# bergmanlab/TELR

Measured on AMD Instinct MI355X. Metric: gbp_aligned_per_s, higher is better.
Workload: dtype int16

## Files before the change

telr_amd/_lib.py:

```python
import ctypes as C
import os
from ._abi import IdxOpt, MapOpt, Aln, Counters, N_STAGES

os.environ.setdefault("GPU_MAX_HW_QUEUES", "2")
_HERE = os.path.dirname(os.path.abspath(__file__))
SO_PATH = os.environ.get("TELR_LIB") or os.path.join(_HERE, "libtelrhip.so")

EXPORTS = [
    "telr_init", "telr_destroy", "telr_strerror", "telr_last_error", "telr_device_name", "telr_preset",
    "telr_seqset_create", "telr_seqset_subset", "telr_seqset_subset_rc", "telr_seqset_free", "telr_seqset_bases", "telr_seqset_count",
    "telr_index_build", "telr_index_free", "telr_index_stats", "telr_map",
    "telr_result_from_arrays", "telr_result_count", "telr_result_alns", "telr_result_cigar_count", "telr_result_cigars", "telr_result_wait", "telr_result_free",
    "telr_init_background", "telr_release_scratch", "telr_device_mem", "telr_write_paf", "telr_write_sam", "telr_write_bam", "telr_write_bam_dev", "telr_bam_prepare", "telr_bam_release_wait", "telr_bam_discard", "telr_write_bam_slice", "telr_bam_segment_info", "telr_bam_segment_entries", "telr_bam_segment_write", "telr_bam_segment_free", "telr_bai_write", "telr_result_from_device_cigars", "telr_seqset_packed", "telr_seqset_from_packed", "telr_consensus_build", "telr_poa_build", "telr_consensus_count", "telr_consensus_seq", "telr_consensus_off", "telr_consensus_len", "telr_consensus_free", "telr_fasta_load", "telr_fasta_count", "telr_fasta_bases", "telr_fasta_extent", "telr_fasta_seq", "telr_fasta_off", "telr_fasta_len", "telr_fasta_names", "telr_fasta_free", "telr_depth_medians", "telr_window_reads", "telr_stage_ms", "telr_stage_name", "telr_last_counters", "telr_last_dp_classes",
]

_lib = None


class TelrError(RuntimeError):
    def __init__(self, msg, code=None):
        RuntimeError.__init__(self, msg)
        self.code = code


# ... 57 lines not shown
        getattr(L, fn).restype = vp; getattr(L, fn).argtypes = [vp]
    L.telr_consensus_free.restype = None; L.telr_consensus_free.argtypes = [vp]
    L.telr_bam_prepare.restype = C.c_int; L.telr_bam_prepare.argtypes = [vp, cp, i64]
    L.telr_bam_release_wait.restype = C.c_int; L.telr_bam_release_wait.argtypes = []
    L.telr_bam_discard.restype = C.c_int; L.telr_bam_discard.argtypes = [vp]
    L.telr_write_bam_slice.restype = C.c_int; L.telr_write_bam_slice.argtypes = [vp, vp, vp, vp, vp, vp, i32, cp, cp, cp, cp, vp, i32, i32, C.POINTER(vp)]
    L.telr_bam_segment_info.restype = C.c_int; L.telr_bam_segment_info.argtypes = [vp, vp]
    L.telr_bam_segment_entries.restype = C.c_int; L.telr_bam_segment_entries.argtypes = [vp, i64, vp, vp, vp, vp, vp]
    L.telr_bam_segment_write.restype = C.c_int; L.telr_bam_segment_write.argtypes = [vp, vp, cp, i64, i32]
    L.telr_bam_segment_free.restype = None; L.telr_bam_segment_free.argtypes = [vp]
    L.telr_bai_write.restype = C.c_int; L.telr_bai_write.argtypes = [cp, i64, vp, vp, vp, vp, C.c_uint64, i64, i32, vp]
    L.telr_result_from_device_cigars.restype = C.c_int; L.telr_result_from_device_cigars.argtypes = [vp, vp, i64, vp, i64, C.POINTER(vp)]
    L.telr_debug_bam_twin.restype = C.c_int; L.telr_debug_bam_twin.argtypes = []
    L.telr_debug_result_twin.restype = i64; L.telr_debug_result_twin.argtypes = [vp, vp, i64]
    L.telr_debug_bam_sink_ms.restype = C.c_int; L.telr_debug_bam_sink_ms.argtypes = [vp]
    L.telr_debug_bam_ms.restype = C.c_int; L.telr_debug_bam_ms.argtypes = [vp]
    L.telr_debug_huff.restype = C.c_int; L.telr_debug_huff.argtypes = [vp, i32, i32, vp]
    L.telr_debug_check_records.restype = C.c_int; L.telr_debug_check_records.argtypes = [vp, i64, vp, i64, vp, i32, vp, i32, C.POINTER(i64)]
    L.telr_debug_deflate_host.restype = C.c_int; L.telr_debug_deflate_host.argtypes = [vp, i32, vp, i32, vp]
    L.telr_stage_ms.restype = C.c_int; L.telr_stage_ms.argtypes = [vp, vp]
    L.telr_stage_name.restype = cp; L.telr_stage_name.argtypes = [C.c_int]
    L.telr_last_counters.restype = C.c_int; L.telr_last_counters.argtypes = [vp, C.POINTER(Counters)]
    L.telr_last_dp_classes.restype = C.c_int; L.telr_last_dp_classes.argtypes = [vp, vp]
    L.telr_debug_n_anchor.restype = i64; L.telr_debug_n_anchor.argtypes = [vp]
    L.telr_debug_dp_retries.restype = i64; L.telr_debug_dp_retries.argtypes = [vp]
    L.telr_debug_pk_launches.restype = i64; L.telr_debug_pk_launches.argtypes = [vp]
    L.telr_debug_fetch.restype = C.c_int; L.telr_debug_fetch.argtypes = [vp, cp, vp, i64]
    L.telr_debug_n_chain.restype = i64; L.telr_debug_n_chain.argtypes = [vp]
    L.telr_debug_chains.restype = vp; L.telr_debug_chains.argtypes = [vp]
    L.telr_debug_index.restype = C.c_int; L.telr_debug_index.argtypes = [vp, vp, vp, vp, vp]
    L.telr_debug_pack.restype = C.c_int; L.telr_debug_pack.argtypes = [cp, i32, C.c_int, vp, vp]
    L.telr_debug_mid_occ.restype = i32; L.telr_debug_mid_occ.argtypes = [vp, C.POINTER(MapOpt)]
    L.telr_debug_dp_limits.restype = C.c_int; L.telr_debug_dp_limits.argtypes = [C.POINTER(MapOpt), vp]
    L.telr_debug_dp.restype = C.c_int; L.telr_debug_dp.argtypes = [vp, vp, vp, C.POINTER(MapOpt), vp, i32, vp, vp, vp, i64]
    L.telr_debug_chain.restype = C.c_int; L.telr_debug_chain.argtypes = [vp, i32, vp, vp, C.POINTER(MapOpt), vp, vp]
    _lib = L
    return L
```

telr_amd/csrc/kernels.hip.h:

```cpp
#pragma once
#include <hip/hip_runtime.h>
#include <stdint.h>

#define TELR_NEG      (-(1 << 28))
#define TELR_TPAD     16384
#define SK_TILE       1024
#define SK_THREADS    256
#define DP_DMAX       4096

struct ChainOpt {
    int32_t max_gap, bw, min_cnt, min_chain_score, chain_gap_q8, chain_skip_q8;
    int32_t dense_n, dense_span, mw_n;
};
struct DpOpt {
    int32_t a, b, q, e, q2, e2, sc_ambi, zdrop;
    int32_t cx_scale, cx_open, cx_emax, cx_emin, cx_dec, cx_flat;
};
__host__ __device__ __forceinline__ int d_cx_ext(const DpOpt &o, int len) { int v = o.cx_emax - o.cx_dec * len; return v > o.cx_emin ? v : o.cx_emin; }
__host__ __device__ __forceinline__ int d_cx_cost(const DpOpt &o, int L)
{
    int t = o.cx_open;
    for (int i = 0; i < L && i < o.cx_flat; ++i) t += d_cx_ext(o, i);
    if (L > o.cx_flat) t += (L - o.cx_flat) * o.cx_emin;
    return t;
// ... 2014 lines not shown
        if (D <= 128) return 6;
        if (D <= 256) return 7;
        if (D <= 512) return 8;
        if (D <= 1024) return 9;
    }
    return D <= 64 ? 0 : D <= 128 ? 1 : D <= 256 ? 2 : D <= 1024 ? 3 : 4;
}
__host__ __device__ __forceinline__ int d_onep_d(int q, int e, int q2, int e2) { return e > e2 ? (q2 - q + (e - e2) - 1) / (e - e2) : 1 << 20; }
__host__ __device__ __forceinline__ bool d_tb4(int cls, int tb4) { return (cls == 17 && (tb4 & 1)) || (cls == 10 && (tb4 & 2)); }
__host__ __device__ __forceinline__ int d_tb4_rowb(int cls) { return cls == 17 ? 8 : 12; }
__host__ __device__ __forceinline__ bool d_tb_tiled(int cls) { return cls == 18 || cls == 23 || cls == 24; }
__device__ __forceinline__ int d_cls_slots(int cls)
{
    if (cls == 22 || cls == 23) return 32;
    if (cls == 24) return 64;
    if (cls >= 19) return 64 << (cls - 19);
    if (cls >= 10) return cls <= 13 ? cls - 5 : cls == 14 ? 10 : cls == 15 ? 12 : cls == 17 ? 4 : 16;
    return cls == 5 ? 32 : 64 << (cls - 6);
}
__device__ __forceinline__ bool d_any_n(const uint32_t *__restrict__ nmask, int64_t lo, int n)
{
    if (n <= 0) return false;
    const int64_t hi = lo + n - 1;
    for (int64_t w = lo >> 5; w <= (hi >> 5); ++w) {
        uint32_t m = nmask[w];
        if (w == (lo >> 5)) m &= ~0u << (int)(lo & 31);
        if (w == (hi >> 5)) m &= ~0u >> (31 - (int)(hi & 31));
        if (m) return true;
    }
    return false;
}
__global__ void k_prob_sizes(DpProb *__restrict__ probs, int32_t np, int fill_margin, int32_t pk_max_steps, int32_t pk_ext_steps, int32_t pk_wide_steps,
                             const uint32_t *__restrict__ qnmask, const uint32_t *__restrict__ tnmask,
                             int64_t *__restrict__ tb_bytes, int64_t *__restrict__ cig_ops, int32_t tb4, int32_t tb4_steps, int32_t pk_wide_maxd, int32_t pk_ext_maxd)
{
    int i = blockIdx.x * blockDim.x + threadIdx.x;
    if (i >= np) return;
    const DpProb P = probs[i];
    int D = P.dhi - P.dlo + 1, stride = (D + 2) / 2;
    int cls = d_dp_class(P.kind, D, P.m + P.n, pk_max_steps, pk_ext_steps, pk_wide_steps, pk_wide_maxd, pk_ext_maxd);
    if (cls >= 10 && P.kind < 3) {
        const bool hasn = d_any_n(qnmask, P.qstep > 0 ? P.qi0 : P.qi0 - P.m + 1, P.m) || d_any_n(tnmask, P.tstep > 0 ? P.ti0 : P.ti0 - P.n + 1, P.n);
        if (hasn) cls = d_dp_class(P.kind, D, P.m + P.n, 0, 0, 0);
    }
    if (d_tb4(cls, tb4) && P.m + P.n > tb4_steps) cls = 14;
    int64_t tb;
    if (P.kind == 5) {
        const int S = P.m < P.n ? P.m : P.n, lm = P.m < S + P.dhi ? P.m : S + P.dhi, ln = P.n < S + P.dhi ? P.n : S + P.dhi;
        tb = (2 * (int64_t)(lm + ln + 1) * (D * 4 + stride) + 127) & ~127LL;
    }
    else if (P.kind >= 3) tb = 0;
    else if (d_tb4(cls, tb4)) tb = ((int64_t)(((P.m + P.n) / 2 + 2) / 2) * (2 * d_tb4_rowb(cls)) + 63) & ~63LL;
    else if (d_tb_tiled(cls)) tb = (int64_t)(((P.m + P.n) / 2 + 4) / 4) * d_cls_slots(cls) * 16;
    else if (cls >= 10) tb = ((int64_t)((P.m + P.n) / 2 + 1) * d_cls_slots(cls) * 4 + 63) & ~63LL;
    else if (cls >= 5) tb = (int64_t)((P.m + P.n) / 4 + 1) * d_cls_slots(cls) * 4;
    else tb = ((int64_t)(P.m + P.n + 1) * stride + 127) & ~127LL;
    int cells = 0;
    if (cls >= 10 && cls != 18 && cls < 23) for (int d = P.dlo; d <= P.dhi; ++d) {
        int ilo = d < 0 ? 1 - d : 1, ihi = P.n - d < P.m ? P.n - d : P.m;
        if (ihi >= ilo) cells += ihi - ilo + 1;
    }
    probs[i].pad[0] = cls | (fill_margin << 8); probs[i].pad[1] = cells;
    tb_bytes[i] = tb;
    if (P.kind == 5) { const int S = P.m < P.n ? P.m : P.n; cig_ops[i] = 3 * (int64_t)(2 * (S + P.dhi) + 2); }
    else cig_ops[i] = P.kind == 3 ? 2 : (int64_t)P.m + P.n;
}
struct ClsOff { int32_t off[DP_NCLS + 1]; };
__device__ __forceinline__ bool d_tb_interleaved(int cls) { return (cls >= 10 && cls <= 13) || cls == 17; }
__device__ __forceinline__ int d_cls_of_pos(const ClsOff &off, int i) { int c = 0; while (c < DP_NCLS - 1 && i >= off.off[c + 1]) ++c; return c; }
__global__ void __launch_bounds__(256) k_tb_gather(const int64_t *__restrict__ tb_bytes, const int32_t *__restrict__ list, int32_t np, ClsOff off, int64_t *__restrict__ out)
{
    const int32_t i = blockIdx.x * blockDim.x + threadIdx.x;
    if (i == np) out[np] = 0;
    if (i >= np) return;
    const int c = d_cls_of_pos(off, i);
    if (!d_tb_interleaved(c)) { out[i] = tb_bytes[list[i]]; return; }
    const int first = off.off[c] + ((i - off.off[c]) & ~63);
    const int last = first + 63 < off.off[c + 1] - 1 ? first + 63 : off.off[c + 1] - 1;
    out[i] = i == last ? tb_bytes[list[first]] * 64 : 0;
}
__global__ void __launch_bounds__(256) k_tb_scatter(DpProb *__restrict__ probs, const int32_t *__restrict__ list, int32_t np, ClsOff off, const int64_t *__restrict__ toff)
{
    const int32_t i = blockIdx.x * blockDim.x + threadIdx.x;
    if (i >= np) return;
    const int c = d_cls_of_pos(off, i);
    probs[list[i]].tb_off = toff[i] + (d_tb_interleaved(c) ? (int64_t)((i - off.off[c]) & 63) * 8 : 0);
}
__global__ void __launch_bounds__(256) k_prob_assign(DpProb *__restrict__ probs, int32_t np, const int64_t *__restrict__ tb_off, const int64_t *__restrict__ cig_off,
                                                     int32_t *__restrict__ cls_cnt, uint32_t *__restrict__ sort_key, int32_t *__restrict__ sort_val)
{
    __shared__ int32_t lcnt[DP_NCLS];
    int i = blockIdx.x * blockDim.x + threadIdx.x;
    if (threadIdx.x < DP_NCLS) lcnt[threadIdx.x] = 0;
    __syncthreads();
    if (i < np) {
        probs[i].tb_off = tb_off[i];
        if (cig_off) probs[i].cig_off = cig_off[i];
        const int c = probs[i].kind >= 3 ? 0 : (probs[i].pad[0] & 0xff);
        atomicAdd(&lcnt[c], 1);
        int steps = probs[i].m + probs[i].n; if (steps > 0x7FFFF) steps = 0x7FFFF;
        sort_key[i] = (uint32_t)c << 19 | (uint32_t)(0x7FFFF - steps);
        sort_val[i] = i;
    }
    __syncthreads();
    if (threadIdx.x < DP_NCLS && lcnt[threadIdx.x]) atomicAdd(&cls_cnt[threadIdx.x], lcnt[threadIdx.x]);
}

__global__ void k_retry_collect(const int32_t *__restrict__ flag, int32_t np, int32_t *__restrict__ cnt, int32_t *__restrict__ list)
{
    const int i = blockIdx.x * blockDim.x + threadIdx.x;
    const bool f = i < np && flag[i];
    const uint64_t m = __ballot(f);
    if (!m) return;
    const int lane = threadIdx.x & 63;
    int base = 0;
    if (lane == __ffsll((unsigned long long)m) - 1) base = atomicAdd(cnt, __popcll(m));
    base = __shfl(base, __ffsll((unsigned long long)m) - 1);
    if (f) list[base + __popcll(m & ((1ULL << lane) - 1))] = i;
}
__global__ void k_retry_build(const DpProb *__restrict__ probs, const int32_t *__restrict__ list, int32_t n, int32_t bw, int32_t band_q4, DpProb *__restrict__ out)
{
    int k = blockIdx.x * blockDim.x + threadIdx.x;
    if (k >= n) return;
    DpProb P = probs[list[k]];
    const int W = d_fill_band(P.m, P.n, bw, band_q4), W2 = d_fill_band_wide(P.m, P.n, bw, band_q4), dl = P.n - P.m;
    const int lo = d_even_lo((dl < 0 ? dl : 0) - W2), hi = (dl > 0 ? dl : 0) + W2;
    P.chain = list[k];
    P.pad[1] = 0;
    if (W2 > W && hi - lo + 1 <= DP_DMAX) { P.dlo = lo; P.dhi = hi; P.kind = 0; } else P.kind = 4;
    out[k] = P;
}
__global__ void k_retry_merge(const DpProb *__restrict__ probs2, const DpRes *__restrict__ res2, int32_t n, DpRes *__restrict__ res)
{
    int k = blockIdx.x * blockDim.x + threadIdx.x;
    if (k >= n || probs2[k].kind == 4) return;
// ... 922 lines not shown
#pragma unroll
                for (int r = 0; r < R; ++r) { REB_ONE(He[r]) REB_ONE(Ho[r]) REB_ONE(E1e[r]) REB_ONE(E1o[r]) REB_ONE(F1e[r]) REB_ONE(F1o[r]) }
#undef REB_ONE
                off += delta;
            }
        }
        if (NW > 1) {
            if (wl == 63) { uint32_t *x = xch + (1 * NW + wv) * 3; x[0] = Ho[R - 1]; x[1] = E1o[R - 1]; x[2] = E2o[R - 1]; }
            __syncthreads();
        }
        if (EXT && __all(done)) break;
    }
    if (EXT) {
        if (have && l == 0) {
            DpRes Rr; Rr.score = best; Rr.bi = bi; Rr.bj = bj; Rr.nops = 0; Rr.mlen = 0; Rr.cells = ncell; Rr.tbases = n; Rr.mcols = 0;
            A.res[prob] = Rr;
        }
        return;
    }
    if (fin_here) {
        int sc = (int)(short)(fin_hi ? (fin >> 16) : (fin & 0xffffu)) + fin_off;
        if constexpr (TB4) sc >>= 2;
        if constexpr (TAG8) sc >>= 3;
        DpRes Rr; Rr.score = sc; Rr.bi = m; Rr.bj = n; Rr.nops = 0; Rr.mlen = 0; Rr.cells = P.pad[1]; Rr.tbases = n; Rr.mcols = 0;
        A.res[prob] = Rr;
    }
}

#define PK_NC 9
__host__ __device__ __forceinline__ int PK_CLS(int c) { return c < 8 ? 10 + c : 22; }
__host__ __device__ __forceinline__ int PK_IDX(int cls) { return cls == 22 ? 8 : cls - 10; }
__device__ __constant__ const int PK_LPP[PK_NC] = { 1, 1, 1, 1, 2, 2, 2, 1, 4 };
__device__ __constant__ const int PK_R[PK_NC]   = { 5, 6, 7, 8, 5, 6, 8, 4, 8 };
struct PkPlan { int32_t woff[PK_NC + 1]; };
__global__ void k_pk_waves(const DpProb *__restrict__ probs, const int32_t *__restrict__ cls_list, ClsOff off, PkPlan plan,
                           uint32_t *__restrict__ keys, uint32_t *__restrict__ vals)
{
    const int i = blockIdx.x * blockDim.x + threadIdx.x;
    if (i >= plan.woff[PK_NC]) return;
    int c = 0;
    while (i >= plan.woff[c + 1]) ++c;
    const int first = (i - plan.woff[c]) * (64 / PK_LPP[c]);
    const DpProb P = probs[cls_list[off.off[PK_CLS(c)] + first]];
    const uint32_t cost = (uint32_t)((P.m + P.n) * PK_R[c]);
    keys[i] = cost > 0xFFFFu ? 0xFFFFu : cost;
    vals[i] = (uint32_t)PK_CLS(c) << 26 | (uint32_t)first;
}
#ifndef PK_WPE
#define PK_WPE 2
#endif
__global__ void __launch_bounds__(64) __attribute__((amdgpu_waves_per_eu(PK_WPE))) k_dp_pk(DpArgs A, const uint32_t *__restrict__ waves, const int32_t *__restrict__ cls_list,
                                              ClsOff off)
{
    const uint32_t w = waves[blockIdx.x];
    const int cls = (int)(w >> 26), first = (int)(w & 0x3ffffffu);
    const int32_t *list = cls_list + off.off[cls];
    const int n = off.off[cls + 1] - off.off[cls];
    if (A.o.cx_scale) {
        switch (cls) {
        case 10: d_dp_pkr<1, 5, false, 1, 4, false, false, false, true>(A, list, n, first); break;
        case 11: d_dp_pkr<1, 6, false, 1, 5, false, false, false, true>(A, list, n, first); break;
        case 12: d_dp_pkr<1, 7, false, 1, 6, false, false, false, true>(A, list, n, first); break;
        case 13: d_dp_pkr<1, 8, false, 1, 7, false, false, false, true>(A, list, n, first); break;
        case 17: d_dp_pkr<1, 4, false, 1, 0, false, false, false, true>(A, list, n, first); break;
        case 14: d_dp_pkr<2, 5, false, 1, 0, false, false, false, true>(A, list, n, first); break;
        case 15: d_dp_pkr<2, 6, false, 1, 0, false, false, false, true>(A, list, n, first); break;
        case 22: d_dp_pkr<4, 8, false, 1, 0, false, false, false, true>(A, list, n, first); break;
        default: d_dp_pkr<2, 8, false, 1, 0, false, false, false, true>(A, list, n, first); break;
        }
        return;
    }
    const int onep_d = d_onep_d(A.o.q, A.o.e, A.o.q2, A.o.e2);
    if (cls == 17 && onep_d >= 16) { if (A.tb4 & 1) d_dp_pkr<1, 4, false, 1, 0, true, true>(A, list, n, first); else d_dp_pkr<1, 4, false, 1, 0, true>(A, list, n, first); return; }
    if (cls == 10 && onep_d >= 20) { if (A.tb4 & 2) d_dp_pkr<1, 5, false, 1, 4, true, true>(A, list, n, first); else d_dp_pkr<1, 5, false, 1, 4, true>(A, list, n, first); return; }
    const DpProb P0 = A.probs[list[first]];
    if (P0.m + P0.n <= A.tag8_steps) {
        switch (cls) {
        case 10: d_dp_pkr<1, 5, false, 1, 4, false, false, true>(A, list, n, first); break;
// ... 564 lines not shown
```

telr_amd/csrc/telr_engine.hip:

```cpp
#include <hip/hip_runtime.h>
#include <cstring>
#include <string.h>
#include <rocprim/rocprim.hpp>
#include <algorithm>
#include <atomic>
#include <immintrin.h>
#include <chrono>
#include <cmath>
#include <condition_variable>
#include <cstdio>
#include <cstdlib>
#include <cstring>
#include <map>
#include <memory>
#include <mutex>
#include <string>
#include <thread>
#include <sys/mman.h>
#include <vector>
#include "../../include/telr_hip.h"
#include "kernels.hip.h"
#define TELR_HAVE_SEED_ARGS 1
#include "segsort.hip.h"
#include "radix.hip.h"
// ... 1267 lines not shown
static inline int tb4_mask(const telr_map_opt *mo)
{
    static const bool off = ab_on("tb_one_launch") || ab_on("tb8");
    if (off || !pk_steps_limit(mo) || mo->cx_scale > 0) return 0;
    const int d = d_onep_d(mo->q, mo->e, mo->q2, mo->e2);
    return (d >= 16 ? 1 : 0) | (d >= 20 ? 2 : 0);
}
static inline int tb4_steps(const telr_map_opt *mo)
{
    const int by_b = 2 * (3850 - mo->q - 32 * mo->e) / (mo->b > 0 ? mo->b : 1) - 2, by_a = 7700 / (mo->a > 0 ? mo->a : 1) - 2;
    const int lim = by_b < by_a ? by_b : by_a;
    return lim > 0 ? lim : 0;
}
static inline int tag8_steps(const telr_map_opt *mo)
{
    static const bool off = ab_on("tb_one_launch") || ab_on("no_tag8");
    if (off || !pk_steps_limit(mo) || mo->cx_scale > 0) return 0;
    const int by_b = 2 * (1975 - mo->q2 - 128 * mo->e2) / (mo->b > 0 ? mo->b : 1) - 2, by_a = 4000 / (mo->a > 0 ? mo->a : 1) - 2;
    const int lim = by_b < by_a ? by_b : by_a;
    return lim > 0 ? lim : 0;
}
static inline int pk_ext_d(const telr_map_opt *mo) { const int D = 2 * mo->ext_band + 2; return D <= 64 ? 64 : D <= 128 ? 128 : 256; }
static inline int pk_ext_limit(const telr_map_opt *mo)
{
    if (!pk_steps_limit(mo) || ab_on("no_pkext")) return 0;
    const int D = pk_ext_d(mo);
    if (mo->cx_scale > 0) return mo->zdrop * mo->cx_scale <= 30000 && pk_cx_ok(mo, D) ? 7900 : 0;
    if (mo->zdrop > 4000) return 0;
    const int by_b = 2 * (15800 - mo->q2 - D * mo->e2) / (mo->b > 0 ? mo->b : 1) - 2, by_a = 32000 / (mo->a > 0 ? mo->a : 1) - 2;
    const int lim = by_b < by_a ? by_b : by_a;
    return lim > 0 ? lim : 0;
}
static inline int pk_ext_maxd(const telr_map_opt *mo) { return pk_ext_limit(mo) ? pk_ext_d(mo) : 64; }
static int dp_pass(telr_ctx *ctx, const telr_seqset *qs, const telr_seqset *tg, const telr_map_opt *mo, DpProb *d_probs, int np, DpRes *d_res,
                   uint32_t **d_rawcig_io, int32_t *d_retry, const std::string &sfx, bool primary)
{
    hipStream_t st = ctx->stream;
    int64_t *d_tbb, *d_cgo, *d_tboff, *d_cgoff; int32_t *d_clscnt, *d_clslist; uint32_t *d_clskey, *d_keytmp; int32_t *d_listtmp;
    ClsOff coff;
    TRY(ctx_buf_t(ctx, ("tb_bytes" + sfx).c_str(), (size_t)np + 1, &d_tbb));
    TRY(ctx_buf_t(ctx, ("cig_ops" + sfx).c_str(), (size_t)np + 1, &d_cgo));
    TRY(ctx_buf_t(ctx, ("tb_off" + sfx).c_str(), (size_t)np + 1, &d_tboff));
    TRY(ctx_buf_t(ctx, ("cig_off" + sfx).c_str(), (size_t)np + 1, &d_cgoff));
    TRY(ctx_buf_t(ctx, ("cls_cnt" + sfx).c_str(), 32, &d_clscnt));
    TRY(ctx_buf_t(ctx, ("cls_list" + sfx).c_str(), (size_t)np, &d_clslist));
    TRY(ctx_buf_t(ctx, ("cls_key" + sfx).c_str(), (size_t)np, &d_clskey));
    TRY(ctx_buf_t(ctx, ("cls_keytmp" + sfx).c_str(), (size_t)np, &d_keytmp));
    TRY(ctx_buf_t(ctx, ("cls_listtmp" + sfx).c_str(), (size_t)np, &d_listtmp));
    hipLaunchKernelGGL(k_prob_sizes, dim3((np + 255) / 256), dim3(256), 0, st, d_probs, np, primary ? mo->fill_margin : 0, pk_steps_limit(mo), pk_ext_limit(mo), pk_wide_limit(mo), qs->d_nmask, tg->d_nmask, d_tbb, d_cgo, tb4_mask(mo), tb4_steps(mo), pk_wide_maxd(mo), pk_ext_maxd(mo));
    HIPCHK(hipGetLastError());
    HIPCHK(hipMemsetAsync(d_tbb + np, 0, 8, st));
    HIPCHK(hipMemsetAsync(d_cgo + np, 0, 8, st));
    TRY((dev_exclusive_scan<int64_t, int64_t>(ctx, d_tbb, d_tboff, (size_t)np + 1)));
    if (primary) TRY((dev_exclusive_scan<int64_t, int64_t>(ctx, d_cgo, d_cgoff, (size_t)np + 1)));
    HIPCHK(hipMemsetAsync(d_clscnt, 0, 128, st));
    hipLaunchKernelGGL(k_prob_assign, dim3((np + 255) / 256), dim3(256), 0, st, d_probs, np, d_tboff, primary ? d_cgoff : (const int64_t*)nullptr, d_clscnt, d_clskey, d_listtmp);
    HIPCHK(hipGetLastError());
    int64_t tb_total = 0, cg_total = 0; int32_t h_cls[32];
    static_assert(DP_NCLS <= 32 && DP_NCLS == TELR_N_DPCLS, "class table");
    HIPCHK(hipMemcpyAsync(&tb_total, d_tboff + np, 8, hipMemcpyDeviceToHost, st));
    if (primary) HIPCHK(hipMemcpyAsync(&cg_total, d_cgoff + np, 8, hipMemcpyDeviceToHost, st));
    HIPCHK(hipMemcpyAsync(h_cls, d_clscnt, 128, hipMemcpyDeviceToHost, st));
    HIPCHK(hipStreamSynchronize(st));
    coff.off[0] = 0;
    for (int c = 0; c < DP_NCLS; ++c) coff.off[c + 1] = coff.off[c] + h_cls[c];
    {
        size_t tbytes = 0;
        HIPCHK(rocprim::radix_sort_pairs(nullptr, tbytes, d_clskey, d_keytmp, d_listtmp, d_clslist, (size_t)np, 0, 24, st));
        void *tmp; TRY(ctx_buf(ctx, "rp_tmp", tbytes, &tmp));
        HIPCHK(rocprim::radix_sort_pairs(tmp, tbytes, d_clskey, d_keytmp, d_listtmp, d_clslist, (size_t)np, 0, 24, st));
    }
    if (np > 0) {
        int64_t *d_tbs;
        TRY(ctx_buf_t(ctx, ("tb_sorted" + sfx).c_str(), (size_t)np + 1, &d_tbs));
        hipLaunchKernelGGL(k_tb_gather, dim3(np / 256 + 1), dim3(256), 0, st, d_tbb, d_clslist, np, coff, d_tbs);
        TRY((dev_exclusive_scan<int64_t, int64_t>(ctx, d_tbs, d_tboff, (size_t)np + 1)));
        hipLaunchKernelGGL(k_tb_scatter, dim3(np / 256 + 1), dim3(256), 0, st, d_probs, d_clslist, np, coff, d_tboff);
        HIPCHK(hipGetLastError());
        HIPCHK(hipMemcpyAsync(&tb_total, d_tboff + np, 8, hipMemcpyDeviceToHost, st));
        HIPCHK(hipStreamSynchronize(st));
    }
    uint8_t *d_tb;
    TRY(ctx_buf_t(ctx, ("tb" + sfx).c_str(), (size_t)tb_total + 256, &d_tb));
    if (primary) TRY(ctx_buf_t(ctx, "rawcig", (size_t)cg_total + 16, d_rawcig_io));
    DpArgs D; D.qseq2 = qs->d_seq2; D.qnmask = qs->d_nmask; D.tseq2 = tg->d_seq2; D.tnmask = tg->d_nmask; D.probs = d_probs;
    D.qtot = qs->padded_bases; D.ttot = tg->padded_bases;
    D.o.a = mo->a; D.o.b = mo->b; D.o.q = mo->q; D.o.e = mo->e; D.o.q2 = mo->q2; D.o.e2 = mo->e2; D.o.sc_ambi = mo->sc_ambi; D.o.zdrop = mo->zdrop;
    D.o.cx_scale = D.o.cx_open = D.o.cx_emax = D.o.cx_emin = D.o.cx_dec = D.o.cx_flat = 0;
    if (mo->cx_scale > 0) {
        const int S = mo->cx_scale;
        D.o.a *= S; D.o.b *= S; D.o.sc_ambi *= S; D.o.zdrop *= S;
        D.o.cx_scale = S; D.o.cx_open = mo->cx_open; D.o.cx_emax = mo->cx_ext_max; D.o.cx_emin = mo->cx_ext_min; D.o.cx_dec = mo->cx_decay;
        D.o.cx_flat = mo->cx_decay > 0 && mo->cx_ext_max > mo->cx_ext_min ? (mo->cx_ext_max - mo->cx_ext_min + mo->cx_decay - 1) / mo->cx_decay : 0;
    }
    D.tb = d_tb; D.cig = *d_rawcig_io; D.res = d_res; D.dcap = 0;
    D.retry = d_retry; D.tb4 = tb4_mask(mo); D.tag8_steps = tag8_steps(mo);
    static const int CAP[5] = { 64, 128, 256, 1024, DP_DMAX };
    static const bool tb_split = !ab_on("tb_one_launch");
    int nw = 0; uint32_t *d_wv2 = nullptr;
    {
        static const int LPP_[PK_NC] = { 1, 1, 1, 1, 2, 2, 2, 1, 4 };
        PkPlan plan; plan.woff[0] = 0;
        for (int c = 0; c < PK_NC; ++c) { const int ppw = 64 / LPP_[c]; plan.woff[c + 1] = plan.woff[c] + (h_cls[PK_CLS(c)] + ppw - 1) / ppw; }
        nw = plan.woff[PK_NC];
        if (nw > 0) {
            uint32_t *d_wk, *d_wv, *d_wk2;
            TRY(ctx_buf_t(ctx, ("pk_wkey" + sfx).c_str(), (size_t)nw, &d_wk));
            TRY(ctx_buf_t(ctx, ("pk_wval" + sfx).c_str(), (size_t)nw, &d_wv));
            TRY(ctx_buf_t(ctx, ("pk_wkey2" + sfx).c_str(), (size_t)nw, &d_wk2));
            TRY(ctx_buf_t(ctx, ("pk_wval2" + sfx).c_str(), (size_t)nw, &d_wv2));
            hipLaunchKernelGGL(k_pk_waves, dim3((nw + 255) / 256), dim3(256), 0, st, d_probs, d_clslist, coff, plan, d_wk, d_wv);
            HIPCHK(hipGetLastError());
            size_t tbytes = 0;
            HIPCHK(rocprim::radix_sort_pairs_desc(nullptr, tbytes, d_wk, d_wk2, d_wv, d_wv2, (size_t)nw, 0, 16, st));
            void *tmp; TRY(ctx_buf(ctx, "rp_tmp", tbytes, &tmp));
            HIPCHK(rocprim::radix_sort_pairs_desc(tmp, tbytes, d_wk, d_wk2, d_wv, d_wv2, (size_t)nw, 0, 16, st));
        }
    }
    HIPCHK(hipEventRecord(ctx->ev_fork, st));
    int side = 0;
    std::vector<hipStream_t> used;
    static const bool serial = getenv("TELR_SERIAL") != nullptr;
    auto side_stream = [&]() { if (serial) return st; hipStream_t s2 = ctx->side[side % TELR_NSIDE]; ++side; used.push_back(s2); return s2; };
    static const int SIDE_ORDER[] = { 9, 4, 3, 21, 8, 20, 24, 23, 18, 2, 7, 19, 1, 0 };
    for (int c : SIDE_ORDER) {
        if (h_cls[c] == 0) continue;
        hipStream_t s2 = side_stream();
        HIPCHK(hipStreamWaitEvent(s2, ctx->ev_fork, 0));
        const int nl = h_cls[c];
        D.list = d_clslist + coff.off[c]; D.nlist = nl; D.dcap = 0;
        if (c <= 4) {
            D.dcap = CAP[c];
            size_t lds = (size_t)(CAP[c] + 2) * 5 * 4;
            static const bool one_wave = ab_on("dp_one_wave");
            if (c >= 3 && !one_wave) {
                if (lds > 48 * 1024) HIPCHK(hipFuncSetAttribute((const void*)k_dp_w4, hipFuncAttributeMaxDynamicSharedMemorySize, (int)lds));
                hipLaunchKernelGGL(k_dp_w4, dim3(nl), dim3(256), lds, s2, D);
            } else {
                if (lds > 48 * 1024) HIPCHK(hipFuncSetAttribute((const void*)k_dp, hipFuncAttributeMaxDynamicSharedMemorySize, (int)lds));
                hipLaunchKernelGGL(k_dp, dim3(nl), dim3(64), lds, s2, D);
            }
        }
        else if (c == 9) hipLaunchKernelGGL((k_dp_reg<256, 2, 4>), dim3(nl), dim3(256), 0, s2, D);
        else if (c == 8) hipLaunchKernelGGL((k_dp_reg<128, 2, 2>), dim3(nl), dim3(128), 0, s2, D);
        else if (c == 7) hipLaunchKernelGGL((k_dp_reg<64, 2>), dim3(nl), dim3(64), 0, s2, D);
        else if (c == 21) hipLaunchKernelGGL((k_dp_pkw<4>), dim3(nl), dim3(256), 0, s2, D);
        else if (c == 20) hipLaunchKernelGGL((k_dp_pkw<2>), dim3(nl), dim3(128), 0, s2, D);
        else if (c == 19) hipLaunchKernelGGL((k_dp_pkw<1>), dim3(nl), dim3(64), 0, s2, D);
        else if (c == 23) { const int ppw = 64 / PKX8_LPP; hipLaunchKernelGGL(k_dp_pkx_w8, dim3((nl + ppw - 1) / ppw), dim3(64), 0, s2, D); }
// ... 444 lines not shown
        }
    });

    const bool do_dp = (mo->flags & TELR_MF_CIGAR) && nk > 0;
    std::vector<int32_t> &h_poff = ctx->h_poffv;
    int64_t *h_foff = nullptr; size_t cig_base = 0; ChainStat *h_cs = nullptr; unsigned long long *h_acc = nullptr;
    int np = 0;
    if (do_dp) {
        StageTimer t_sg(ctx, ST_SEGMENTS, true);
        int32_t *d_nprob, *d_poff;
        TRY(ctx_buf_t(ctx, "nprob", (size_t)nk + 1, &d_nprob));
        TRY(ctx_buf_t(ctx, "prob_off", (size_t)nk + 1, &d_poff));
        hipLaunchKernelGGL(k_segments_w<0>, dim3(nk), dim3(64), 0, st, d_kc, nk, d_canch, mo->min_ksw_len, mo->bw, mo->fill_band_q4, mo->ext_max, mo->ext_band, mo->bw_long, d_nprob, (const int32_t*)nullptr, (DpProb*)nullptr);
        HIPCHK(hipGetLastError());
        HIPCHK(hipMemsetAsync(d_nprob + nk, 0, 4, st));
        TRY((dev_exclusive_scan<int32_t, int32_t>(ctx, d_nprob, d_poff, (size_t)nk + 1)));
        h_poff.resize(nk + 1);
        HIPCHK(hipMemcpyAsync(h_poff.data(), d_poff, (size_t)(nk + 1) * 4, hipMemcpyDeviceToHost, st));
        HIPCHK(hipStreamSynchronize(st));
        np = h_poff[nk];
        DpProb *d_probs;
        TRY(ctx_buf_t(ctx, "probs", (size_t)np, &d_probs));
        hipLaunchKernelGGL(k_segments_w<1>, dim3(nk), dim3(64), 0, st, d_kc, nk, d_canch, mo->min_ksw_len, mo->bw, mo->fill_band_q4, mo->ext_max, mo->ext_band, mo->bw_long, d_nprob, d_poff, d_probs);
        HIPCHK(hipGetLastError());
        t_sg.stop(); ht.mark("segments (sync: problems)");
        ctx->ctr.dp_problems += np;

        StageTimer t_dp(ctx, ST_DP, true);
        uint32_t *d_rawcig = nullptr; DpRes *d_res; int32_t *d_retry, *d_rcnt, *d_rlist;
        TRY(ctx_buf_t(ctx, "dp_res", (size_t)np, &d_res));
        TRY(ctx_buf_t(ctx, "retry_flag", (size_t)np + 1, &d_retry));
        TRY(ctx_buf_t(ctx, "retry_list", (size_t)np + 1, &d_rlist));
        TRY(ctx_buf_t(ctx, "retry_cnt", 4, &d_rcnt));
        HIPCHK(hipMemsetAsync(d_retry, 0, ((size_t)np + 1) * 4, st));
        HIPCHK(hipMemsetAsync(d_rcnt, 0, 16, st));
        TRY(dp_pass(ctx, qs, tg, mo, d_probs, np, d_res, &d_rawcig, d_retry, "", true));
        hipLaunchKernelGGL(k_retry_collect, dim3((np + 255) / 256), dim3(256), 0, st, d_retry, np, d_rcnt, d_rlist);
        HIPCHK(hipGetLastError());
        int32_t n_retry = 0;
        HIPCHK(hipMemcpyAsync(&n_retry, d_rcnt, 4, hipMemcpyDeviceToHost, st));
        HIPCHK(hipStreamSynchronize(st));
        { float ms = 0;
          if (hipEventElapsedTime(&ms, ctx->evk[5], ctx->evk[0]) == hipSuccess) ctx->stage_ms[ST_K_PK] += ms;
          if (hipEventElapsedTime(&ms, ctx->evk[0], ctx->evk[1]) == hipSuccess) ctx->stage_ms[ST_K_REG] += ms;
          if (hipEventElapsedTime(&ms, ctx->evk[3], ctx->evk[4]) == hipSuccess) ctx->stage_ms[ST_K_TRACEBACK] += ms; }
        if (n_retry > 0) {
            DpProb *d_probs2; DpRes *d_res2;
            TRY(ctx_buf_t(ctx, "probs_r", (size_t)n_retry, &d_probs2));
            TRY(ctx_buf_t(ctx, "dp_res_r", (size_t)n_retry, &d_res2));
            hipLaunchKernelGGL(k_retry_build, dim3((n_retry + 255) / 256), dim3(256), 0, st, d_probs, d_rlist, n_retry, mo->bw, mo->fill_band_q4, d_probs2);
            HIPCHK(hipGetLastError());
            TRY(dp_pass(ctx, qs, tg, mo, d_probs2, n_retry, d_res2, &d_rawcig, nullptr, "_r", false));
            hipLaunchKernelGGL(k_retry_merge, dim3((n_retry + 255) / 256), dim3(256), 0, st, d_probs2, d_res2, n_retry, d_res);
            HIPCHK(hipGetLastError());
        }
        ctx->dp_retries += n_retry;
        t_dp.stop(); ht.mark("dp passes");

        StageTimer t_g(ctx, ST_GATHER, true);
        {
            StitchRec *h_sv, *d_sv; int64_t *d_nfin, *d_foff; StitchProb *d_sp;
            TRY(ctx_hbuf_t(ctx, "h_stitch", (size_t)nk, &h_sv));
            TRY(ctx_buf_t(ctx, "stitch", (size_t)nk, &d_sv));
            TRY(ctx_buf_t(ctx, "stitch_n", (size_t)nk + 1, &d_nfin));
            TRY(ctx_buf_t(ctx, "stitch_off", (size_t)nk + 1, &d_foff));
            TRY(ctx_buf_t(ctx, "stitch_prob", (size_t)np, &d_sp));
            parallel_ranges(NT, nk, [&](int, int xa, int xb) {
// ... 386 lines not shown
    *needed = out_off[n_win];
    if (*needed > cap) return TELR_E_RANGE;
    for (int w = 0; w < n_win; ++w) if (len_of[w]) memcpy(out_qid + out_off[w], all.data() + src_of[w], (size_t)len_of[w] * 4);
    return TELR_OK;
}

extern "C" int64_t telr_debug_dp_retries(const telr_ctx *ctx) { return ctx ? ctx->dp_retries : 0; }
extern "C" int64_t telr_debug_pk_launches(const telr_ctx *ctx) { return ctx ? ctx->pk_launches : 0; }
extern "C" int64_t telr_debug_n_anchor(const telr_ctx *ctx) { return ctx ? ctx->dbg_na : 0; }
extern "C" int telr_debug_fetch(telr_ctx *ctx, const char *what, void *dst, int64_t bytes)
{
    if (!ctx || !what || !dst) return TELR_E_ARG;
    auto it = ctx->bufs.find(what);
    if (it == ctx->bufs.end() || !it->second.p || (size_t)bytes > it->second.bytes) return TELR_E_ARG;
    HIPCHK(hipMemcpy(dst, it->second.p, (size_t)bytes, hipMemcpyDeviceToHost));
    return TELR_OK;
}
extern "C" int64_t telr_debug_n_chain(const telr_ctx *ctx) { return ctx ? (int64_t)ctx->dbg_chain.size() / 9 : 0; }
extern "C" const int32_t *telr_debug_chains(const telr_ctx *ctx) { return ctx ? ctx->dbg_chain.data() : nullptr; }
extern "C" int telr_debug_index(telr_ctx *ctx, const telr_index *ix, uint64_t *ent_hash, uint32_t *ent_off, uint32_t *pos)
{
    if (!ctx || !ix) return TELR_E_ARG;
    if (ent_hash) HIPCHK(hipMemcpy(ent_hash, ix->d_ent_hash, (size_t)ix->n_ent * 8, hipMemcpyDeviceToHost));
    if (ent_off) HIPCHK(hipMemcpy(ent_off, ix->d_ent_off, ((size_t)ix->n_ent + 1) * 4, hipMemcpyDeviceToHost));
    if (pos) HIPCHK(hipMemcpy(pos, ix->d_pos, (size_t)ix->n_mz * 4, hipMemcpyDeviceToHost));
    return TELR_OK;
}
extern "C" int32_t telr_debug_mid_occ(const telr_index *ix, const telr_map_opt *mo) { return ix && mo ? index_mid_occ(ix, mo) : -1; }
extern "C" int telr_debug_dp_limits(const telr_map_opt *mo, int32_t *out)
{
    if (!mo || !out) return TELR_E_ARG;
    out[0] = pk_steps_limit(mo); out[1] = pk_wide_limit(mo); out[2] = pk_wide_maxd(mo); out[3] = pk_ext_limit(mo);
    out[4] = pk_ext_maxd(mo); out[5] = tb4_mask(mo); out[6] = tb4_steps(mo); out[7] = tag8_steps(mo);
    return TELR_OK;
}
extern "C" int telr_debug_chain(telr_ctx *ctx, int32_t nq, const uint64_t *keys, const int32_t *q_aoff, const telr_map_opt *mo, int32_t *f, int32_t *p)
{
    (void)hipGetLastError();
    if (!ctx || !mo || nq < 0 || nq > (1 << 24) || (nq > 0 && !q_aoff)) return TELR_E_ARG;
    TRY(check_map_opt(ctx, mo));
    if (nq == 0) return TELR_OK;
    if (q_aoff[0] != 0) { ctx->err = "telr_debug_chain: q_aoff[0] must be 0"; return TELR_E_ARG; }
    int32_t n_over = 0;
    std::vector<int32_t> over;
    for (int q = 0; q < nq; ++q) {
        const int32_t a0 = q_aoff[q], a1 = q_aoff[q + 1];
        if (a1 < a0 || a1 > (1 << 30)) { ctx->err = "telr_debug_chain: q_aoff must ascend (at most 2^30 anchors)"; return TELR_E_ARG; }
        for (int32_t i = a0 + 1; i < a1; ++i)
            if (keys[i] < keys[i - 1]) { ctx->err = "telr_debug_chain: the anchors of query " + std::to_string(q) + " are not sorted"; return TELR_E_ARG; }
        if (a1 - a0 > SEGSORT_CAP) { over.push_back(q); ++n_over; }
    }
    const int32_t na = q_aoff[nq];
    if (na > 0 && (!keys || !f || !p)) return TELR_E_ARG;
    if (na == 0) return TELR_OK;
    HIPCHK(hipSetDevice(ctx->device));
    hipStream_t st = ctx->stream;
    uint64_t *d_keys; int32_t *d_qaoff, *d_over, *d_f, *d_p;
    TRY(ctx_buf_t(ctx, "dbg_ch_keys", (size_t)na, &d_keys));
    TRY(ctx_buf_t(ctx, "dbg_ch_qaoff", (size_t)nq + 1, &d_qaoff));
    TRY(ctx_buf_t(ctx, "dbg_ch_over", (size_t)n_over + 1, &d_over));
    TRY(ctx_buf_t(ctx, "dbg_ch_f", (size_t)na, &d_f));
    TRY(ctx_buf_t(ctx, "dbg_ch_p", (size_t)na, &d_p));
    HIPCHK(hipMemcpyAsync(d_keys, keys, (size_t)na * 8, hipMemcpyHostToDevice, st));
    HIPCHK(hipMemcpyAsync(d_qaoff, q_aoff, ((size_t)nq + 1) * 4, hipMemcpyHostToDevice, st));
    if (n_over) HIPCHK(hipMemcpyAsync(d_over, over.data(), (size_t)n_over * 4, hipMemcpyHostToDevice, st));
    TRY(chain_dispatch(ctx, st, mo, d_keys, d_qaoff, nq, na, n_over, d_over, nullptr, d_f, d_p));
// ... 552 lines not shown
```

Measured before the change: 20.65.

## Replace DP class and wave radix sorts with hashed counting sort

After: 20.06. 2.9% lower.

```diff
diff --git a/telr_amd/_lib.py b/telr_amd/_lib.py
--- a/telr_amd/_lib.py
+++ b/telr_amd/_lib.py
@@ -113,6 +113,8 @@
     L.telr_debug_pack.restype = C.c_int; L.telr_debug_pack.argtypes = [cp, i32, C.c_int, vp, vp]
     L.telr_debug_mid_occ.restype = i32; L.telr_debug_mid_occ.argtypes = [vp, C.POINTER(MapOpt)]
     L.telr_debug_dp_limits.restype = C.c_int; L.telr_debug_dp_limits.argtypes = [C.POINTER(MapOpt), vp]
+    if hasattr(L, "telr_debug_dp_order"):
+        L.telr_debug_dp_order.restype = C.c_int; L.telr_debug_dp_order.argtypes = [C.POINTER(MapOpt), vp, vp, i32, vp, vp, vp]
     L.telr_debug_dp.restype = C.c_int; L.telr_debug_dp.argtypes = [vp, vp, vp, C.POINTER(MapOpt), vp, i32, vp, vp, vp, i64]
     L.telr_debug_chain.restype = C.c_int; L.telr_debug_chain.argtypes = [vp, i32, vp, vp, C.POINTER(MapOpt), vp, vp]
     _lib = L
diff --git a/telr_amd/csrc/kernels.hip.h b/telr_amd/csrc/kernels.hip.h
--- a/telr_amd/csrc/kernels.hip.h
+++ b/telr_amd/csrc/kernels.hip.h
@@ -2070,10 +2070,13 @@
 }
 __global__ void k_prob_sizes(DpProb *__restrict__ probs, int32_t np, int fill_margin, int32_t pk_max_steps, int32_t pk_ext_steps, int32_t pk_wide_steps,
                              const uint32_t *__restrict__ qnmask, const uint32_t *__restrict__ tnmask,
-                             int64_t *__restrict__ tb_bytes, int64_t *__restrict__ cig_ops, int32_t tb4, int32_t tb4_steps, int32_t pk_wide_maxd, int32_t pk_ext_maxd)
+                             int64_t *__restrict__ tb_bytes, int64_t *__restrict__ cig_ops, int32_t tb4, int32_t tb4_steps, int32_t pk_wide_maxd, int32_t pk_ext_maxd,
+                             int32_t *__restrict__ retry)
 {
     int i = blockIdx.x * blockDim.x + threadIdx.x;
+    if (i == 0) { tb_bytes[np] = 0; cig_ops[np] = 0; }
     if (i >= np) return;
+    if (retry) retry[i] = 0;
     const DpProb P = probs[i];
     int D = P.dhi - P.dlo + 1, stride = (D + 2) / 2;
     int cls = d_dp_class(P.kind, D, P.m + P.n, pk_max_steps, pk_ext_steps, pk_wide_steps, pk_wide_maxd, pk_ext_maxd);
@@ -2104,6 +2107,71 @@
     else cig_ops[i] = P.kind == 3 ? 2 : (int64_t)P.m + P.n;
 }
 struct ClsOff { int32_t off[DP_NCLS + 1]; };
+#define CLS_STEP_BINS 8192
+#define CLS_NBIN (DP_NCLS * CLS_STEP_BINS)
+#define CSORT_TILE 4096
+#define CSORT_SLOTS 2048
+#define CSORT_PROBES 8
+#define CSORT_EMPTY 0xffffffffu
+__host__ __device__ __forceinline__ uint32_t d_cls_bin(int cls, int steps)
+{
+    const int s = steps < CLS_STEP_BINS - 1 ? steps : CLS_STEP_BINS - 1;
+    return (uint32_t)(cls * CLS_STEP_BINS + (CLS_STEP_BINS - 1 - s));
+}
+template <bool INSERT>
+__device__ __forceinline__ int d_csort_slot(uint32_t *hk, uint32_t b)
+{
+    const uint32_t h = (b * 2654435761u) >> 21;
+    static_assert(CSORT_SLOTS == 2048, "hash width");
+    for (int p = 0; p < CSORT_PROBES; ++p) {
+        const int s = (int)((h + p) & (CSORT_SLOTS - 1));
+        const uint32_t prev = INSERT ? atomicCAS(&hk[s], CSORT_EMPTY, b) : hk[s];
+        if (prev == b || (INSERT && prev == CSORT_EMPTY)) return s;
+    }
+    return -1;
+}
+__device__ __forceinline__ void d_csort_count(const uint32_t *__restrict__ bin, int32_t n, uint32_t *hk, int32_t *hc, int32_t *__restrict__ direct)
+{
+    const int tid = threadIdx.x;
+    for (int s = tid; s < CSORT_SLOTS; s += 256) { hk[s] = CSORT_EMPTY; hc[s] = 0; }
+    __syncthreads();
+    const int64_t base = (int64_t)blockIdx.x * CSORT_TILE;
+    for (int j = 0; j < CSORT_TILE / 256; ++j) {
+        const int64_t i = base + j * 256 + tid;
+        if (i >= n) break;
+        const uint32_t b = bin[i];
+        const int s = d_csort_slot<true>(hk, b);
+        if (s >= 0) atomicAdd(&hc[s], 1);
+        else if (direct) atomicAdd(&direct[b], 1);
+    }
+    __syncthreads();
+}
+__global__ void __launch_bounds__(256) k_csort_hist(const uint32_t *__restrict__ bin, int32_t n, int32_t *__restrict__ hist)
+{
+    __shared__ uint32_t hk[CSORT_SLOTS];
+    __shared__ int32_t hc[CSORT_SLOTS];
+    d_csort_count(bin, n, hk, hc, hist);
+    for (int s = threadIdx.x; s < CSORT_SLOTS; s += 256) if (hc[s]) atomicAdd(&hist[hk[s]], hc[s]);
+}
+__global__ void __launch_bounds__(256) k_csort_scatter(const uint32_t *__restrict__ bin, const uint32_t *__restrict__ vals, int32_t n, int32_t *__restrict__ cursor,
+                                                       uint32_t *__restrict__ out)
+{
+    __shared__ uint32_t hk[CSORT_SLOTS];
+    __shared__ int32_t hc[CSORT_SLOTS];
+    d_csort_count(bin, n, hk, hc, nullptr);
+    for (int s = threadIdx.x; s < CSORT_SLOTS; s += 256) if (hc[s]) hc[s] = atomicAdd(&cursor[hk[s]], hc[s]);
+    __syncthreads();
+    const int tid = threadIdx.x;
+    const int64_t base = (int64_t)blockIdx.x * CSORT_TILE;
+    for (int j = 0; j < CSORT_TILE / 256; ++j) {
+        const int64_t i = base + j * 256 + tid;
+        if (i >= n) break;
+        const uint32_t b = bin[i];
+        const int s = d_csort_slot<false>(hk, b);
+        const int32_t at = s >= 0 ? atomicAdd(&hc[s], 1) : atomicAdd(&cursor[b], 1);
+        out[at] = vals ? vals[i] : (uint32_t)i;
+    }
+}
 __device__ __forceinline__ bool d_tb_interleaved(int cls) { return (cls >= 10 && cls <= 13) || cls == 17; }
 __device__ __forceinline__ int d_cls_of_pos(const ClsOff &off, int i) { int c = 0; while (c < DP_NCLS - 1 && i >= off.off[c + 1]) ++c; return c; }
 __global__ void __launch_bounds__(256) k_tb_gather(const int64_t *__restrict__ tb_bytes, const int32_t *__restrict__ list, int32_t np, ClsOff off, int64_t *__restrict__ out)
@@ -2125,11 +2193,13 @@
     probs[list[i]].tb_off = toff[i] + (d_tb_interleaved(c) ? (int64_t)((i - off.off[c]) & 63) * 8 : 0);
 }
 __global__ void __launch_bounds__(256) k_prob_assign(DpProb *__restrict__ probs, int32_t np, const int64_t *__restrict__ tb_off, const int64_t *__restrict__ cig_off,
-                                                     int32_t *__restrict__ cls_cnt, uint32_t *__restrict__ sort_key, int32_t *__restrict__ sort_val)
+                                                     int32_t *__restrict__ cls_cnt, uint32_t *__restrict__ sort_key, int32_t *__restrict__ sort_val,
+                                                     int32_t *__restrict__ bin_hist)
 {
     __shared__ int32_t lcnt[DP_NCLS];
     int i = blockIdx.x * blockDim.x + threadIdx.x;
     if (threadIdx.x < DP_NCLS) lcnt[threadIdx.x] = 0;
+    if (bin_hist) for (int j = i; j < CLS_NBIN; j += gridDim.x * blockDim.x) bin_hist[j] = 0;
     __syncthreads();
     if (i < np) {
         probs[i].tb_off = tb_off[i];
@@ -2137,8 +2207,11 @@
         const int c = probs[i].kind >= 3 ? 0 : (probs[i].pad[0] & 0xff);
         atomicAdd(&lcnt[c], 1);
         int steps = probs[i].m + probs[i].n; if (steps > 0x7FFFF) steps = 0x7FFFF;
-        sort_key[i] = (uint32_t)c << 19 | (uint32_t)(0x7FFFF - steps);
-        sort_val[i] = i;
+        if (bin_hist) sort_key[i] = d_cls_bin(c, steps);
+        else {
+            sort_key[i] = (uint32_t)c << 19 | (uint32_t)(0x7FFFF - steps);
+            sort_val[i] = i;
+        }
     }
     __syncthreads();
     if (threadIdx.x < DP_NCLS && lcnt[threadIdx.x]) atomicAdd(&cls_cnt[threadIdx.x], lcnt[threadIdx.x]);
@@ -3127,18 +3200,21 @@
 __host__ __device__ __forceinline__ int PK_IDX(int cls) { return cls == 22 ? 8 : cls - 10; }
 __device__ __constant__ const int PK_LPP[PK_NC] = { 1, 1, 1, 1, 2, 2, 2, 1, 4 };
 __device__ __constant__ const int PK_R[PK_NC]   = { 5, 6, 7, 8, 5, 6, 8, 4, 8 };
+#define PK_WBINS 1024
+__host__ __device__ __forceinline__ uint32_t d_pk_wave_bin(uint32_t cost) { return PK_WBINS - 1 - ((cost > 0xFFFFu ? 0xFFFFu : cost) >> 6); }
 struct PkPlan { int32_t woff[PK_NC + 1]; };
 __global__ void k_pk_waves(const DpProb *__restrict__ probs, const int32_t *__restrict__ cls_list, ClsOff off, PkPlan plan,
-                           uint32_t *__restrict__ keys, uint32_t *__restrict__ vals)
+                           uint32_t *__restrict__ keys, uint32_t *__restrict__ vals, int32_t *__restrict__ bin_hist)
 {
     const int i = blockIdx.x * blockDim.x + threadIdx.x;
+    if (bin_hist) for (int j = i; j < PK_WBINS; j += gridDim.x * blockDim.x) bin_hist[j] = 0;
     if (i >= plan.woff[PK_NC]) return;
     int c = 0;
     while (i >= plan.woff[c + 1]) ++c;
     const int first = (i - plan.woff[c]) * (64 / PK_LPP[c]);
     const DpProb P = probs[cls_list[off.off[PK_CLS(c)] + first]];
     const uint32_t cost = (uint32_t)((P.m + P.n) * PK_R[c]);
-    keys[i] = cost > 0xFFFFu ? 0xFFFFu : cost;
+    keys[i] = bin_hist ? d_pk_wave_bin(cost) : cost > 0xFFFFu ? 0xFFFFu : cost;
     vals[i] = (uint32_t)PK_CLS(c) << 26 | (uint32_t)first;
 }
 #ifndef PK_WPE
diff --git a/telr_amd/csrc/telr_engine.hip b/telr_amd/csrc/telr_engine.hip
--- a/telr_amd/csrc/telr_engine.hip
+++ b/telr_amd/csrc/telr_engine.hip
@@ -1323,6 +1323,15 @@
     return lim > 0 ? lim : 0;
 }
 static inline int pk_ext_maxd(const telr_map_opt *mo) { return pk_ext_limit(mo) ? pk_ext_d(mo) : 64; }
+static inline bool dp_order_fits(const telr_map_opt *mo)
+{
+    return pk_steps_limit(mo) < CLS_STEP_BINS && pk_ext_limit(mo) < CLS_STEP_BINS && pk_wide_limit(mo) < CLS_STEP_BINS;
+}
+static inline bool dp_order_by_count(const telr_map_opt *mo)
+{
+    static const bool on = ab_on("dp_order_count") && !ab_on("dp_sort_lib");
+    return on && dp_order_fits(mo);
+}
 static int dp_pass(telr_ctx *ctx, const telr_seqset *qs, const telr_seqset *tg, const telr_map_opt *mo, DpProb *d_probs, int np, DpRes *d_res,
                    uint32_t **d_rawcig_io, int32_t *d_retry, const std::string &sfx, bool primary)
 {
@@ -1338,15 +1347,25 @@
     TRY(ctx_buf_t(ctx, ("cls_key" + sfx).c_str(), (size_t)np, &d_clskey));
     TRY(ctx_buf_t(ctx, ("cls_keytmp" + sfx).c_str(), (size_t)np, &d_keytmp));
     TRY(ctx_buf_t(ctx, ("cls_listtmp" + sfx).c_str(), (size_t)np, &d_listtmp));
-    hipLaunchKernelGGL(k_prob_sizes, dim3((np + 255) / 256), dim3(256), 0, st, d_probs, np, primary ? mo->fill_margin : 0, pk_steps_limit(mo), pk_ext_limit(mo), pk_wide_limit(mo), qs->d_nmask, tg->d_nmask, d_tbb, d_cgo, tb4_mask(mo), tb4_steps(mo), pk_wide_maxd(mo), pk_ext_maxd(mo));
+    hipLaunchKernelGGL(k_prob_sizes, dim3((np + 255) / 256), dim3(256), 0, st, d_probs, np, primary ? mo->fill_margin : 0, pk_steps_limit(mo), pk_ext_limit(mo), pk_wide_limit(mo), qs->d_nmask, tg->d_nmask, d_tbb, d_cgo, tb4_mask(mo), tb4_steps(mo), pk_wide_maxd(mo), pk_ext_maxd(mo), d_retry);
     HIPCHK(hipGetLastError());
-    HIPCHK(hipMemsetAsync(d_tbb + np, 0, 8, st));
-    HIPCHK(hipMemsetAsync(d_cgo + np, 0, 8, st));
     TRY((dev_exclusive_scan<int64_t, int64_t>(ctx, d_tbb, d_tboff, (size_t)np + 1)));
     if (primary) TRY((dev_exclusive_scan<int64_t, int64_t>(ctx, d_cgo, d_cgoff, (size_t)np + 1)));
     HIPCHK(hipMemsetAsync(d_clscnt, 0, 128, st));
-    hipLaunchKernelGGL(k_prob_assign, dim3((np + 255) / 256), dim3(256), 0, st, d_probs, np, d_tboff, primary ? d_cgoff : (const int64_t*)nullptr, d_clscnt, d_clskey, d_listtmp);
+    const bool by_count = dp_order_by_count(mo);
+    int32_t *d_binhist = nullptr, *d_bincur = nullptr;
+    if (by_count) {
+        TRY(ctx_buf_t(ctx, ("cls_binhist" + sfx).c_str(), (size_t)CLS_NBIN, &d_binhist));
+        TRY(ctx_buf_t(ctx, ("cls_bincur" + sfx).c_str(), (size_t)CLS_NBIN + 1, &d_bincur));
+    }
+    hipLaunchKernelGGL(k_prob_assign, dim3((np + 255) / 256), dim3(256), 0, st, d_probs, np, d_tboff, primary ? d_cgoff : (const int64_t*)nullptr, d_clscnt, d_clskey, d_listtmp, d_binhist);
     HIPCHK(hipGetLastError());
+    if (by_count && np > 0) {
+        hipLaunchKernelGGL(k_csort_hist, dim3((np + CSORT_TILE - 1) / CSORT_TILE), dim3(256), 0, st, d_clskey, np, d_binhist);
+        TRY((dev_qscan<int32_t, int32_t>(ctx, d_binhist, CLS_NBIN, d_bincur, nullptr, 0, nullptr, nullptr)));
+        hipLaunchKernelGGL(k_csort_scatter, dim3((np + CSORT_TILE - 1) / CSORT_TILE), dim3(256), 0, st, d_clskey, (const uint32_t*)nullptr, np, d_bincur, (uint32_t*)d_clslist);
+        HIPCHK(hipGetLastError());
+    }
     int64_t tb_total = 0, cg_total = 0; int32_t h_cls[32];
     static_assert(DP_NCLS <= 32 && DP_NCLS == TELR_N_DPCLS, "class table");
     HIPCHK(hipMemcpyAsync(&tb_total, d_tboff + np, 8, hipMemcpyDeviceToHost, st));
@@ -1355,7 +1374,7 @@
     HIPCHK(hipStreamSynchronize(st));
     coff.off[0] = 0;
     for (int c = 0; c < DP_NCLS; ++c) coff.off[c + 1] = coff.off[c] + h_cls[c];
-    {
+    if (!by_count) {
         size_t tbytes = 0;
         HIPCHK(rocprim::radix_sort_pairs(nullptr, tbytes, d_clskey, d_keytmp, d_listtmp, d_clslist, (size_t)np, 0, 24, st));
         void *tmp; TRY(ctx_buf(ctx, "rp_tmp", tbytes, &tmp));
@@ -1400,12 +1419,24 @@
             TRY(ctx_buf_t(ctx, ("pk_wval" + sfx).c_str(), (size_t)nw, &d_wv));
             TRY(ctx_buf_t(ctx, ("pk_wkey2" + sfx).c_str(), (size_t)nw, &d_wk2));
             TRY(ctx_buf_t(ctx, ("pk_wval2" + sfx).c_str(), (size_t)nw, &d_wv2));
-            hipLaunchKernelGGL(k_pk_waves, dim3((nw + 255) / 256), dim3(256), 0, st, d_probs, d_clslist, coff, plan, d_wk, d_wv);
+            int32_t *d_whist = nullptr, *d_wcur = nullptr;
+            if (by_count) {
+                TRY(ctx_buf_t(ctx, ("pk_whist" + sfx).c_str(), (size_t)PK_WBINS, &d_whist));
+                TRY(ctx_buf_t(ctx, ("pk_wcur" + sfx).c_str(), (size_t)PK_WBINS + 1, &d_wcur));
+            }
+            hipLaunchKernelGGL(k_pk_waves, dim3((nw + 255) / 256), dim3(256), 0, st, d_probs, d_clslist, coff, plan, d_wk, d_wv, d_whist);
             HIPCHK(hipGetLastError());
-            size_t tbytes = 0;
-            HIPCHK(rocprim::radix_sort_pairs_desc(nullptr, tbytes, d_wk, d_wk2, d_wv, d_wv2, (size_t)nw, 0, 16, st));
-            void *tmp; TRY(ctx_buf(ctx, "rp_tmp", tbytes, &tmp));
-            HIPCHK(rocprim::radix_sort_pairs_desc(tmp, tbytes, d_wk, d_wk2, d_wv, d_wv2, (size_t)nw, 0, 16, st));
+            if (by_count) {
+                hipLaunchKernelGGL(k_csort_hist, dim3((nw + CSORT_TILE - 1) / CSORT_TILE), dim3(256), 0, st, d_wk, nw, d_whist);
+                TRY((dev_qscan<int32_t, int32_t>(ctx, d_whist, PK_WBINS, d_wcur, nullptr, 0, nullptr, nullptr)));
+                hipLaunchKernelGGL(k_csort_scatter, dim3((nw + CSORT_TILE - 1) / CSORT_TILE), dim3(256), 0, st, d_wk, d_wv, nw, d_wcur, d_wv2);
+                HIPCHK(hipGetLastError());
+            } else {
+                size_t tbytes = 0;
+                HIPCHK(rocprim::radix_sort_pairs_desc(nullptr, tbytes, d_wk, d_wk2, d_wv, d_wv2, (size_t)nw, 0, 16, st));
+                void *tmp; TRY(ctx_buf(ctx, "rp_tmp", tbytes, &tmp));
+                HIPCHK(rocprim::radix_sort_pairs_desc(tmp, tbytes, d_wk, d_wk2, d_wv, d_wv2, (size_t)nw, 0, 16, st));
+            }
         }
     }
     HIPCHK(hipEventRecord(ctx->ev_fork, st));
@@ -1916,7 +1947,6 @@
         TRY(ctx_buf_t(ctx, "retry_flag", (size_t)np + 1, &d_retry));
         TRY(ctx_buf_t(ctx, "retry_list", (size_t)np + 1, &d_rlist));
         TRY(ctx_buf_t(ctx, "retry_cnt", 4, &d_rcnt));
-        HIPCHK(hipMemsetAsync(d_retry, 0, ((size_t)np + 1) * 4, st));
         HIPCHK(hipMemsetAsync(d_rcnt, 0, 16, st));
         TRY(dp_pass(ctx, qs, tg, mo, d_probs, np, d_res, &d_rawcig, d_retry, "", true));
         hipLaunchKernelGGL(k_retry_collect, dim3((np + 255) / 256), dim3(256), 0, st, d_retry, np, d_rcnt, d_rlist);
@@ -2369,6 +2399,17 @@
     if (!mo || !out) return TELR_E_ARG;
     out[0] = pk_steps_limit(mo); out[1] = pk_wide_limit(mo); out[2] = pk_wide_maxd(mo); out[3] = pk_ext_limit(mo);
     out[4] = pk_ext_maxd(mo); out[5] = tb4_mask(mo); out[6] = tb4_steps(mo); out[7] = tag8_steps(mo);
+    return TELR_OK;
+}
+extern "C" int telr_debug_dp_order(const telr_map_opt *mo, const int32_t *cls, const int32_t *steps, int32_t n, int32_t *bin, int32_t *wave_bin, int32_t *by_count)
+{
+    if (!mo || n < 0 || (n > 0 && (!cls || !steps || !bin || !wave_bin)) || !by_count) return TELR_E_ARG;
+    for (int i = 0; i < n; ++i) {
+        if (cls[i] < 0 || cls[i] >= DP_NCLS || steps[i] < 0) return TELR_E_ARG;
+        bin[i] = (int32_t)d_cls_bin(cls[i], steps[i] > 0x7FFFF ? 0x7FFFF : steps[i]);
+        wave_bin[i] = (int32_t)d_pk_wave_bin((uint32_t)steps[i] * 8u);
+    }
+    by_count[0] = dp_order_fits(mo) ? 1 : 0; by_count[1] = CLS_STEP_BINS; by_count[2] = PK_WBINS;
     return TELR_OK;
 }
 extern "C" int telr_debug_chain(telr_ctx *ctx, int32_t nq, const uint64_t *keys, const int32_t *q_aoff, const telr_map_opt *mo, int32_t *f, int32_t *p)
```
